# zjwfufu/FateAvatar

Measured on AMD Instinct MI355X. Metric: render+backward frames/sec at 512^2, 100k Gaussians, higher is better.
Workload: dtype f32

## Files before the change

### fateavatar_amd/csrc/fr_common.hpp

```cpp
#pragma once
#include <hip/hip_runtime.h>
#include <stdint.h>
#include <stddef.h>
#include <vector>
#include "../../include/fr_rasterizer.h"

namespace fr {

constexpr int kWave = 64;
constexpr int kTile = 8;
constexpr int kRefTile = 16;
constexpr int kAccumStride = 16;
constexpr int kXcds = 8;
constexpr int kSubWords = 8;
constexpr uint32_t kDensePairsFwd = 1000;
constexpr uint32_t kDensePairsBwd = 1000;
#ifndef FR_PRE_WG
#define FR_PRE_WG 128
#endif
constexpr int kPreWG = FR_PRE_WG;
constexpr uint32_t kBucketCapInit = 64;
constexpr int kSortWaveMax = 256;
constexpr int kSortGroupMax = 2048;
constexpr int kSortRegMax = 4096;
// ... 344 lines not shown
int launch_l1_loss_grad(unsigned long long n, const float* img, const float* gt, float* grad, float* loss, void* workspace,
                        hipStream_t s);
int launch_l1_loss_grad_terms(int n_images, unsigned long long n, float rgb_weight, const float* const* img, const float* const* gt,
                              float* const* grad, float* const* loss, void* const* workspace, hipStream_t s);
void ssim_window(float out[11]);
size_t image_loss_workspace_bytes(int C, int H, int W);
int launch_image_loss_grad(const fr_image_loss_config& cfg, int n_images, int C, int H, int W, const float* const* img,
                           const float* const* gt, float* const* grad, float* const* loss, void* const* workspace, hipStream_t s);
int launch_scaled_sum(int n_src, const float* const* src, float* dst, unsigned long long count, float scale, hipStream_t s);
size_t regularise_workspace_bytes();
int launch_gaussian_regularise(const fr_regularise_config& cfg, int P, const float* scaling, const float* xyz, float* d_scaling,
                               float* d_xyz, float* loss, void* workspace, hipStream_t s);
int launch_multi_copy(int n_seg, float* const* dst, const float* const* src, const unsigned long long* count, hipStream_t s);
int launch_selftest_reduce(const float* in, float* out, hipStream_t s);

#if defined(__HIPCC__)
__device__ __forceinline__ float act_sigmoid(float x) { return 1.0f / (1.0f + expf(-x)); }
__device__ __forceinline__ float act_exp(float x) { return expf(x); }
__device__ __forceinline__ float act_rot_inv_norm(float r, float x, float y, float z)
{
    return 1.0f / fmaxf(sqrtf(r * r + x * x + y * y + z * z), 1e-12f);
}

__device__ __forceinline__ void cov3d_from_scale_rot(float sc0, float sc1, float sc2, float r, float x, float y, float z,
                                                     float scale_modifier, float (&c3)[6])
{
    const float s0 = scale_modifier * sc0, s1 = scale_modifier * sc1, s2 = scale_modifier * sc2;
    const float m00 = s0 * (1.f - 2.f * (y * y + z * z)), m01 = s1 * (2.f * (x * y - r * z)), m02 = s2 * (2.f * (x * z + r * y));
    const float m10 = s0 * (2.f * (x * y + r * z)), m11 = s1 * (1.f - 2.f * (x * x + z * z)), m12 = s2 * (2.f * (y * z - r * x));
    const float m20 = s0 * (2.f * (x * z - r * y)), m21 = s1 * (2.f * (y * z + r * x)), m22 = s2 * (1.f - 2.f * (x * x + y * y));
    c3[0] = m00 * m00 + m01 * m01 + m02 * m02;
    c3[1] = m10 * m00 + m11 * m01 + m12 * m02;
    c3[2] = m20 * m00 + m21 * m01 + m22 * m02;
    c3[3] = m10 * m10 + m11 * m11 + m12 * m12;
    c3[4] = m20 * m10 + m21 * m11 + m22 * m12;
    c3[5] = m20 * m20 + m21 * m21 + m22 * m22;
}
constexpr unsigned kDoneGroups = 16, kDoneStride = 32;
__device__ __forceinline__ bool last_workgroup_of(unsigned* c, unsigned id, unsigned count)
{
    const unsigned groups = count < kDoneGroups ? count : kDoneGroups;
    const unsigned g = id % groups;
    const unsigned members = (count - g + groups - 1u) / groups;
    if (atomicInc(c + g * kDoneStride, members - 1u) != members - 1u) return false;
    return atomicInc(c + kDoneGroups * kDoneStride, groups - 1u) == groups - 1u;
}
__device__ __forceinline__ int lane_id() { return (int)__builtin_amdgcn_mbcnt_hi(~0u, __builtin_amdgcn_mbcnt_lo(~0u, 0u)); }

__device__ __forceinline__ void atomic_add_f32(float* p, float v) { unsafeAtomicAdd(p, v); }

struct CameraRegs {
    float view[16], proj[16], campos[3];
};
__device__ __forceinline__ CameraRegs load_camera(const float* view, const float* proj, const float* campos, int lane)
{
    float x = 0.f;
    if (lane < 16) x = view[lane];
    else if (lane < 32) x = proj[lane - 16];
    else if (lane < 35) x = campos[lane - 32];
    const int xi = __float_as_int(x);
    CameraRegs c;
#pragma unroll
    for (int k = 0; k < 16; k++) {
        c.view[k] = __int_as_float(__builtin_amdgcn_readlane(xi, k));
        c.proj[k] = __int_as_float(__builtin_amdgcn_readlane(xi, 16 + k));
    }
#pragma unroll
    for (int k = 0; k < 3; k++) c.campos[k] = __int_as_float(__builtin_amdgcn_readlane(xi, 32 + k));
    return c;
}

__device__ __forceinline__ float3 xform4x3(const float3 p, const float* m)
{
    return make_float3(m[0] * p.x + m[4] * p.y + m[8] * p.z + m[12], m[1] * p.x + m[5] * p.y + m[9] * p.z + m[13],
                       m[2] * p.x + m[6] * p.y + m[10] * p.z + m[14]);
}
__device__ __forceinline__ float4 xform4x4(const float3 p, const float* m)
{
    return make_float4(m[0] * p.x + m[4] * p.y + m[8] * p.z + m[12], m[1] * p.x + m[5] * p.y + m[9] * p.z + m[13],
                       m[2] * p.x + m[6] * p.y + m[10] * p.z + m[14], m[3] * p.x + m[7] * p.y + m[11] * p.z + m[15]);
}
#endif

}
```

### fateavatar_amd/csrc/fr_preprocess.hip

```cpp
#include "fr_bind_math.hpp"

#ifdef FR_DIAG_PRE_ABLATE
#define FR_PRE_ABLATE(k) (((FR_DIAG_PRE_ABLATE) >> (k)) & 1)
#else
#define FR_PRE_ABLATE(k) false
#endif

#ifdef FR_DIAG_PRE_TRACE
namespace fr {
constexpr unsigned kPreTraceWaves = 16384, kPreTraceSlots = 12;
__device__ unsigned long long g_pre_trace[kPreTraceWaves * kPreTraceSlots];
}
extern "C" int fr_diag_read_pre_trace(void* dst, size_t bytes)
{
    return (int)hipMemcpyFromSymbol(dst, HIP_SYMBOL(fr::g_pre_trace), bytes < sizeof(fr::g_pre_trace) ? bytes : sizeof(fr::g_pre_trace));
}
#define PRE_TR_DECL unsigned long long ptr_acc[::fr::kPreTraceSlots] = {0, 0, 0, 0, 0, 0, 0, 0, 0, 0, 0, 0}, ptr_t = __builtin_readcyclecounter(), ptr_rt0 = __builtin_amdgcn_s_memrealtime()
#define PRE_TR(k) do { const unsigned long long n_ = __builtin_readcyclecounter(); ptr_acc[(k)] += n_ - ptr_t; ptr_t = n_; } while (0)
#define PRE_TR_STORE() do { \
        ptr_acc[11] = (ptr_rt0 << 32) | (__builtin_amdgcn_s_memrealtime() & 0xFFFFFFFFull); \
        const unsigned w_ = (blockIdx.x * kPreWG + threadIdx.x) >> 6; \
        if (lane == 0 && w_ < ::fr::kPreTraceWaves && blockIdx.y == 0) \
            for (unsigned k_ = 0; k_ < ::fr::kPreTraceSlots; k_++) ::fr::g_pre_trace[(size_t)w_ * ::fr::kPreTraceSlots + k_] = ptr_acc[k_]; \
    } while (0)
// ... 98 lines not shown


__device__ __forceinline__ bool footprint_touches_tile(const float4 conic_tau2, const float2 ctr, uint32_t tx, uint32_t ty)
{
    if (!(conic_tau2.w < 3.0e38f)) return true;
    const float A = conic_tau2.x, B = conic_tau2.y, C = conic_tau2.z, t2 = conic_tau2.w;
    const float lox = (float)(tx * kTile) - ctr.x, hix = lox + (float)(kTile - 1);
    const float loy = (float)(ty * kTile) - ctr.y, hiy = loy + (float)(kTile - 1);
    const float qx = lox > 0.f ? lox : (hix < 0.f ? hix : 0.f);
    const float qy = loy > 0.f ? loy : (hiy < 0.f ? hiy : 0.f);
    if (qx == 0.f && qy == 0.f) return true;
    const float dy = fminf(fmaxf(-B * qx * __builtin_amdgcn_rcpf(C), loy), hiy);
    const float dx = fminf(fmaxf(-B * qy * __builtin_amdgcn_rcpf(A), lox), hix);
    const float ax = A * qx * qx, bx = 2.f * B * qx * dy, cx = C * dy * dy;
    const float ay = A * dx * dx, by = 2.f * B * dx * qy, cy = C * qy * qy;
    const float q1 = (ax + bx) + cx, m1 = (ax + fabsf(bx)) + cx;
    const float q2 = (ay + by) + cy, m2 = (ay + fabsf(by)) + cy;
    const bool in1 = qx != 0.f && q1 <= t2 + (4.0e-6f * m1 + 1.0e-4f);
    const bool in2 = qy != 0.f && q2 <= t2 + (4.0e-6f * m2 + 1.0e-4f);
    return in1 || in2;
}

constexpr int kCountUnroll = 4;
constexpr int kCountLdsBytes = 2816 + 3 * kCountUnroll * 256;

#ifndef FR_PRE_SH_DMA
#define FR_PRE_SH_DMA 2
#endif
__device__ __forceinline__ void dma16_to_lds(const void* g, uint32_t lds_byte_address )
{
    asm volatile("s_mov_b32 m0, %0\n\ts_nop 0\n\tglobal_load_lds_dwordx4 %1, off" ::"s"(lds_byte_address), "v"(g) : "memory");
}
#ifndef FR_PRE_ROWS_IN_REGS
#define FR_PRE_ROWS_IN_REGS 1
#endif
__host__ __device__ constexpr int pre_wave_lds_bytes(int M3)
{
#if FR_PRE_ROWS_IN_REGS
    if (M3 == 48) return 256 * M3;
#endif
    return 256 * M3 + kCountLdsBytes;
}

template <bool FWD_ONLY>
__device__ __forceinline__ void preprocess_fwd_body(const PreArgs& a)
{
    extern __shared__ __attribute__((aligned(16))) float s_sh[];
    const int idx = blockIdx.x * blockDim.x + threadIdx.x;
    const int lane = threadIdx.x & 63, wave = threadIdx.x >> 6;
    if (blockIdx.x == 0 && threadIdx.x < sizeof(DeviceCounts) / 4) reinterpret_cast<uint32_t*>(a.counts)[threadIdx.x] = 0u;
    if ((int)(blockIdx.x * kPreWG) >= a.P) return;
    const int M3 = a.M * 3;
    PRE_TR_DECL;
    const CameraRegs cam = load_camera(a.view, a.proj, a.campos, lane);
    const bool live = idx < a.P;
    const int li = live ? idx : 0;
    float3 p_orig;
    float in_sc[3] = {0.f, 0.f, 0.f}, in_rot[4] = {0.f, 0.f, 0.f, 0.f};
    if (a.bound) {
        float bp[3];
        bind_fwd(a.bind, li, bp, in_rot, in_sc);
        p_orig = make_float3(bp[0], bp[1], bp[2]);
        if (live) {
            float* m = const_cast<float*>(a.means3D) + 3 * (size_t)li;
            float* r = const_cast<float*>(a.rotations) + 4 * (size_t)li;
            float* sc = const_cast<float*>(a.scales) + 3 * (size_t)li;
            m[0] = bp[0], m[1] = bp[1], m[2] = bp[2];
            r[0] = in_rot[0], r[1] = in_rot[1], r[2] = in_rot[2], r[3] = in_rot[3];
            sc[0] = in_sc[0], sc[1] = in_sc[1], sc[2] = in_sc[2];
        }
    } else {
        p_orig = make_float3(a.means3D[3 * li], a.means3D[3 * li + 1], a.means3D[3 * li + 2]);
        if (a.scales) in_sc[0] = a.scales[3 * li], in_sc[1] = a.scales[3 * li + 1], in_sc[2] = a.scales[3 * li + 2];
        if (a.rotations)
            in_rot[0] = a.rotations[4 * li], in_rot[1] = a.rotations[4 * li + 1], in_rot[2] = a.rotations[4 * li + 2],
            in_rot[3] = a.rotations[4 * li + 3];
    }
    const float in_opacity = a.opacities[li];
    float in_col[3] = {0.f, 0.f, 0.f};
    if (a.colors_precomp) in_col[0] = a.colors_precomp[3 * li], in_col[1] = a.colors_precomp[3 * li + 1], in_col[2] = a.colors_precomp[3 * li + 2];
    float* const wave_lds = s_sh + (size_t)wave * (pre_wave_lds_bytes(M3) / 4);
    const int wave_first = blockIdx.x * kPreWG + wave * 64;
    const bool rows_in_lds = a.shs && !a.colors_precomp && !FR_PRE_ABLATE(0);
    const bool sh_in_lds = rows_in_lds && __builtin_amdgcn_readfirstlane((int)(FR_PRE_SH_DMA && wave_first + 64 <= a.P)) != 0;
#if FR_PRE_SH_DMA
    if (sh_in_lds) {
        const char* blk = reinterpret_cast<const char*>(a.shs + (size_t)wave_first * M3);
        const int bytes = 256 * M3;
#if FR_PRE_SH_DMA == 2
        const uint32_t lds0 = (uint32_t)__builtin_amdgcn_readfirstlane(
            (int)(uintptr_t)(__attribute__((address_space(3))) void*)wave_lds);
#endif
        for (int off = 0; off < bytes; off += 1024)
            if (off + lane * 16 < bytes) {
#if FR_PRE_SH_DMA == 2
                dma16_to_lds(blk + off + lane * 16, lds0 + (uint32_t)off);
#else
                __builtin_amdgcn_global_load_lds((const __attribute__((address_space(1))) void*)(blk + off + lane * 16),
                                                 (__attribute__((address_space(3))) void*)(reinterpret_cast<char*>(wave_lds) + off), 16, 0, 0);
#endif
            }
    }
#endif
    if (rows_in_lds && !sh_in_lds && live)
        for (int k = 0; k < M3; k++) wave_lds[lane * M3 + k] = a.shs[(size_t)idx * M3 + k];
    uint32_t ref_tiles = 0;
    uint2 rect = make_uint2(0u, 0u);
    float4 cull = make_float4(0.f, 0.f, 0.f, __builtin_inff());
    float2 ctr = make_float2(0.f, 0.f);
    bool alive = false;
    int mr_out = 0;
    float rec_ca = 0.f, rec_cb = 0.f, rec_cc = 0.f, rec_op = 0.f, rec_z = 0.f;
    PRE_TR(0);
    if (idx < a.P) {
        do {
            const float3 p_view = xform4x3(p_orig, cam.view);
            PRE_TR(1);
            if (p_view.z <= 0.2f) break;
            if (FR_PRE_ABLATE(5) && in_opacity > -1e30f) break;

            const float4 p_hom = xform4x4(p_orig, cam.proj);
            const float p_w = 1.0f / (p_hom.w + 0.0000001f);
            const float p_proj_x = p_hom.x * p_w, p_proj_y = p_hom.y * p_w;

            float c3[6];
            if (a.cov3D_precomp) {
                for (int k = 0; k < 6; k++) c3[k] = a.cov3D_precomp[6 * (size_t)idx + k];
            } else {
                float sc0 = in_sc[0], sc1 = in_sc[1], sc2 = in_sc[2];
                float r = in_rot[0], x = in_rot[1], y = in_rot[2], z = in_rot[3];
                if (a.raw) {
                    sc0 = act_exp(sc0), sc1 = act_exp(sc1), sc2 = act_exp(sc2);
                    const float inv = act_rot_inv_norm(r, x, y, z);
// ... 621 lines not shown
```

### fateavatar_amd/csrc/fr_preprocess_bwd.hip

```cpp
#include "fr_bind_math.hpp"

namespace fr {

__constant__ float bSH_C0 = 0.28209479177387814f;
__constant__ float bSH_C1 = 0.4886025119029199f;
__constant__ float bSH_C2[5] = {1.0925484305920792f, -1.0925484305920792f, 0.31539156525252005f,
                                -1.0925484305920792f, 0.5462742152960396f};
__constant__ float bSH_C3[7] = {-0.5900435899266435f, 2.890611442640554f, -0.4570457994644658f, 0.3731763325901154f,
                                -0.4570457994644658f, 1.445305721320277f,  -0.5900435899266435f};

struct PreBwdArgs {
    int P, D, M, W, H, raw;
    float tan_fovx, tan_fovy, focal_x, focal_y, scale_modifier;
    const float* means3D;
    const float* scales;
    const float* rotations;
    const float* shs;
    const float* cov3D_precomp;
    const float* view;
    const float* proj;
    const float* campos;
    const int* radii;
    GeomView g;
    fr_grads out;
    float* grad_accum;
    float* denom;
    float* overflow_out;
    const DeviceCounts* counts;
    uint32_t acc;
    int bound;
    BindArgs bind;
    BindGrads bg;
};

enum { G_MEANS2D = 0, G_COLORS, G_OPACITY, G_MEANS3D, G_COV3D, G_SH, G_SCALES, G_ROTATIONS };

__device__ __forceinline__ void put(float* p, float v, bool add) { *p = add ? *p + v : v; }

__device__ __forceinline__ void store3(float* p, size_t i, float a, float b, float c, bool add)
{
    if (!p) return;
    if (add) a += p[3 * i], b += p[3 * i + 1], c += p[3 * i + 2];
    p[3 * i] = a, p[3 * i + 1] = b, p[3 * i + 2] = c;
}

template <bool PLANES>
__device__ __forceinline__ void preprocess_bwd_one(const PreBwdArgs& a, const CameraRegs& cam, const int radius,
                                                   const int idx, float* row)
{
    const size_t i = (size_t)idx;
    const int Mc = a.M;
    const auto adds = [&](int k) { return ((a.acc >> k) & 1u) != 0u; };
    if (!(radius > 0)) {
        if (row)
            for (int k = 0; k < Mc * 3; k++) row[k] = 0.f;
        if (!adds(G_MEANS2D)) store3(a.out.dL_dmeans2D, i, 0.f, 0.f, 0.f, false);
        if (!adds(G_COLORS)) store3(a.out.dL_dcolors, i, 0.f, 0.f, 0.f, false);
        if (a.out.dL_dopacity && !adds(G_OPACITY)) a.out.dL_dopacity[i] = 0.f;
        if (!adds(G_MEANS3D)) store3(a.out.dL_dmeans3D, i, 0.f, 0.f, 0.f, false);
        if (a.out.dL_dcov3D && !adds(G_COV3D))
            for (int k = 0; k < 6; k++) a.out.dL_dcov3D[6 * i + k] = 0.f;
        if (a.out.dL_dsh && !row && !adds(G_SH))
            for (int k = 0; k < Mc * 3; k++) a.out.dL_dsh[i * Mc * 3 + k] = 0.f;
        if (!adds(G_SCALES)) store3(a.out.dL_dscales, i, 0.f, 0.f, 0.f, false);
        if (a.out.dL_drotations && !adds(G_ROTATIONS))
            for (int k = 0; k < 4; k++) a.out.dL_drotations[4 * i + k] = 0.f;
        if (a.bound) bind_bwd_zero(idx, a.bg);
        return;
    }
    float old_m3[3] = {0.f, 0.f, 0.f}, old_sc[3] = {0.f, 0.f, 0.f}, old_q[4] = {0.f, 0.f, 0.f, 0.f}, old_op = 0.f;
    if (a.acc) {
        if (adds(G_MEANS3D) && a.out.dL_dmeans3D)
            for (int k = 0; k < 3; k++) old_m3[k] = a.out.dL_dmeans3D[3 * i + k];
        if (adds(G_SCALES) && a.out.dL_dscales)
            for (int k = 0; k < 3; k++) old_sc[k] = a.out.dL_dscales[3 * i + k];
        if (adds(G_ROTATIONS) && a.out.dL_drotations)
            for (int k = 0; k < 4; k++) old_q[k] = a.out.dL_drotations[4 * i + k];
        if (adds(G_OPACITY) && a.out.dL_dopacity) old_op = a.out.dL_dopacity[i];
    }
    float acc[12];
    {
        float4* row4 = reinterpret_cast<float4*>(a.g.accum + i * kAccumStride);
        const float4 r0 = row4[0], r1 = row4[1], r2 = row4[2];
        row4[0] = row4[1] = row4[2] = make_float4(0.f, 0.f, 0.f, 0.f);
        acc[0] = r0.x, acc[1] = r0.y, acc[2] = r0.z, acc[3] = r0.w, acc[4] = r1.x, acc[5] = r1.y, acc[6] = r1.z,
        acc[7] = r1.w, acc[8] = r2.x, acc[9] = r2.y, acc[10] = r2.z, acc[11] = r2.w;
    }
    const float3 mean = make_float3(a.means3D[3 * idx], a.means3D[3 * idx + 1], a.means3D[3 * idx + 2]);
    const float* vm = cam.view;
    float q_r = 0.f, q_x = 0.f, q_y = 0.f, q_z = 0.f, rot_inv = 1.0f;
    float sc[3] = {0.f, 0.f, 0.f};
    float c3[6];
    if (a.scales) {
        q_r = a.rotations[4 * idx], q_x = a.rotations[4 * idx + 1], q_y = a.rotations[4 * idx + 2], q_z = a.rotations[4 * idx + 3];
        sc[0] = a.scales[3 * idx], sc[1] = a.scales[3 * idx + 1], sc[2] = a.scales[3 * idx + 2];
        if (a.raw) {
            sc[0] = act_exp(sc[0]), sc[1] = act_exp(sc[1]), sc[2] = act_exp(sc[2]);
            rot_inv = act_rot_inv_norm(q_r, q_x, q_y, q_z);
            q_r *= rot_inv, q_x *= rot_inv, q_y *= rot_inv, q_z *= rot_inv;
        }
    }
    if (a.cov3D_precomp) {
        for (int k = 0; k < 6; k++) c3[k] = a.cov3D_precomp[6 * i + k];
    } else {
        cov3d_from_scale_rot(sc[0], sc[1], sc[2], q_r, q_x, q_y, q_z, a.scale_modifier, c3);
    }

    float3 t = xform4x3(mean, vm);
    const float limx = 1.3f * a.tan_fovx, limy = 1.3f * a.tan_fovy;
    const float txtz = t.x / t.z, tytz = t.y / t.z;
    t.x = fminf(limx, fmaxf(-limx, txtz)) * t.z;
    t.y = fminf(limy, fmaxf(-limy, tytz)) * t.z;
    const float x_grad_mul = txtz < -limx || txtz > limx ? 0 : 1;
    const float y_grad_mul = tytz < -limy || tytz > limy ? 0 : 1;
    const float h_x = a.focal_x, h_y = a.focal_y;
    const float j00 = h_x / t.z, j02 = -(h_x * t.x) / (t.z * t.z);
    const float j11 = h_y / t.z, j12 = -(h_y * t.y) / (t.z * t.z);
    float T0[3], T1[3];
    for (int w = 0; w < 3; w++) {
        const float W0 = vm[4 * w], W1 = vm[4 * w + 1], W2 = vm[4 * w + 2];
        T0[w] = W0 * j00 + W1 * 0.0f + W2 * j02;
        T1[w] = W0 * 0.0f + W1 * j11 + W2 * j12;
    }
    const float V[3][3] = {{c3[0], c3[1], c3[2]}, {c3[1], c3[3], c3[4]}, {c3[2], c3[4], c3[5]}};
    float A0[3], A1[3];
    for (int c = 0; c < 3; c++) {
        A0[c] = T0[0] * V[0][c] + T0[1] * V[1][c] + T0[2] * V[2][c];
        A1[c] = T1[0] * V[0][c] + T1[1] * V[1][c] + T1[2] * V[2][c];
    }
    float ca = A0[0] * T0[0] + A0[1] * T0[1] + A0[2] * T0[2];
    const float cb = A1[0] * T0[0] + A1[1] * T0[1] + A1[2] * T0[2];
    float cc = A1[0] * T1[0] + A1[1] * T1[1] + A1[2] * T1[2];
    ca += 0.3f;
    cc += 0.3f;
    const float denom = ca * cc - cb * cb;
    const float det_inv = 1.f / denom;
    const float4 co = make_float4(cc * det_inv, -cb * det_inv, ca * det_inv, a.g.opacity_act[idx]);
    const float g2x = acc[ACC_MX] * (0.5f * a.W);
    const float g2y = acc[ACC_MY] * (0.5f * a.H);
    const float dcx = -0.5f * acc[ACC_CA], dcy = -0.5f * acc[ACC_CB], dcz = -0.5f * acc[ACC_CC];
    const float dop = (co.w != 0.f) ? acc[ACC_OP] / co.w : 0.f;
    float dcol[3] = {acc[ACC_R], acc[ACC_G], acc[ACC_B]};
    store3(a.out.dL_dmeans2D, i, g2x, g2y, 0.f, adds(G_MEANS2D));
    if (!a.counts->overflow) {
        if (a.grad_accum) a.grad_accum[i] += sqrtf(g2x * g2x + g2y * g2y);
        if (a.denom) a.denom[i] += 1.0f;
    }
    store3(a.out.dL_dcolors, i, dcol[0], dcol[1], dcol[2], adds(G_COLORS));
    if (a.out.dL_dopacity) a.out.dL_dopacity[i] = old_op + (a.raw ? dop * co.w * (1.0f - co.w) : dop);

    float dL_da = 0, dL_db = 0, dL_dc = 0;
    const float denom2inv = 1.0f / ((denom * denom) + 0.0000001f);
    float dcov[6] = {0, 0, 0, 0, 0, 0};
    if (denom2inv != 0) {
        dL_da = denom2inv * (-cc * cc * dcx + 2 * cb * cc * dcy + (denom - ca * cc) * dcz);
        dL_dc = denom2inv * (-ca * ca * dcz + 2 * ca * cb * dcy + (denom - ca * cc) * dcx);
        dL_db = denom2inv * 2 * (cb * cc * dcx - (denom + 2 * cb * cb) * dcy + ca * cb * dcz);
        dcov[0] = (T0[0] * T0[0] * dL_da + T0[0] * T1[0] * dL_db + T1[0] * T1[0] * dL_dc);
        dcov[3] = (T0[1] * T0[1] * dL_da + T0[1] * T1[1] * dL_db + T1[1] * T1[1] * dL_dc);
        dcov[5] = (T0[2] * T0[2] * dL_da + T0[2] * T1[2] * dL_db + T1[2] * T1[2] * dL_dc);
        dcov[1] = 2 * T0[0] * T0[1] * dL_da + (T0[0] * T1[1] + T0[1] * T1[0]) * dL_db + 2 * T1[0] * T1[1] * dL_dc;
        dcov[2] = 2 * T0[0] * T0[2] * dL_da + (T0[0] * T1[2] + T0[2] * T1[0]) * dL_db + 2 * T1[0] * T1[2] * dL_dc;
        dcov[4] = 2 * T0[2] * T0[1] * dL_da + (T0[1] * T1[2] + T0[2] * T1[1]) * dL_db + 2 * T1[1] * T1[2] * dL_dc;
    }
    if (a.out.dL_dcov3D)
        for (int k = 0; k < 6; k++) put(a.out.dL_dcov3D + 6 * i + k, dcov[k], adds(G_COV3D));

    float dT0[3], dT1[3];
    for (int c = 0; c < 3; c++) {
        const float tv0 = T0[0] * V[c][0] + T0[1] * V[c][1] + T0[2] * V[c][2];
        const float tv1 = T1[0] * V[c][0] + T1[1] * V[c][1] + T1[2] * V[c][2];
        dT0[c] = 2 * tv0 * dL_da + tv1 * dL_db;
        dT1[c] = 2 * tv1 * dL_dc + tv0 * dL_db;
    }
    const float dL_dJ00 = vm[0] * dT0[0] + vm[4] * dT0[1] + vm[8] * dT0[2];
    const float dL_dJ02 = vm[2] * dT0[0] + vm[6] * dT0[1] + vm[10] * dT0[2];
    const float dL_dJ11 = vm[1] * dT1[0] + vm[5] * dT1[1] + vm[9] * dT1[2];
    const float dL_dJ12 = vm[2] * dT1[0] + vm[6] * dT1[1] + vm[10] * dT1[2];
    const float tz = 1.f / t.z, tz2 = tz * tz, tz3 = tz2 * tz;
    const float dL_dtx = x_grad_mul * -h_x * tz2 * dL_dJ02;
    const float dL_dty = y_grad_mul * -h_y * tz2 * dL_dJ12;
    const float dL_dtz = -h_x * tz2 * dL_dJ00 - h_y * tz2 * dL_dJ11 + (2 * h_x * t.x) * tz3 * dL_dJ02 + (2 * h_y * t.y) * tz3 * dL_dJ12;
    float dmx = vm[0] * dL_dtx + vm[1] * dL_dty + vm[2] * dL_dtz;
    float dmy = vm[4] * dL_dtx + vm[5] * dL_dty + vm[6] * dL_dtz;
    float dmz = vm[8] * dL_dtx + vm[9] * dL_dty + vm[10] * dL_dtz;

    {
        const float* proj = cam.proj;
        const float4 m_hom = xform4x4(mean, proj);
        const float m_w = 1.0f / (m_hom.w + 0.0000001f);
        const float mul1 = (proj[0] * mean.x + proj[4] * mean.y + proj[8] * mean.z + proj[12]) * m_w * m_w;
        const float mul2 = (proj[1] * mean.x + proj[5] * mean.y + proj[9] * mean.z + proj[13]) * m_w * m_w;
        const float px = (proj[0] * m_w - proj[3] * mul1) * g2x + (proj[1] * m_w - proj[3] * mul2) * g2y;
        const float py = (proj[4] * m_w - proj[7] * mul1) * g2x + (proj[5] * m_w - proj[7] * mul2) * g2y;
        const float pz = (proj[8] * m_w - proj[11] * mul1) * g2x + (proj[9] * m_w - proj[11] * mul2) * g2y;
        dmx += px, dmy += py, dmz += pz;
    }

    if (a.shs) {
        const float dox = mean.x - cam.campos[0], doy = mean.y - cam.campos[1], doz = mean.z - cam.campos[2];
        const float len = sqrtf(dox * dox + doy * doy + doz * doz);
        const float x = dox / len, y = doy / len, z = doz / len;
        const uint8_t cl = a.g.clamped[idx];
        float dRGB[3];
        for (int c = 0; c < 3; c++) dRGB[c] = dcol[c] * (((cl >> c) & 1) ? 0 : 1);
        const float* dd = a.g.dcolor_ddir + i * 9;
        const float dRGBdx[3] = {dd[0], dd[1], dd[2]}, dRGBdy[3] = {dd[3], dd[4], dd[5]}, dRGBdz[3] = {dd[6], dd[7], dd[8]};
        const int deg = a.D;
        const int used = (deg + 1) * (deg + 1);
        auto write_row = [&](float* dsh, const bool dsh_adds) {
#define DSH(k, c, v_) put(dsh + (k) * 3 + (c), (v_), dsh_adds)
            for (int c = 0; c < 3; c++) {
                DSH(0, c, bSH_C0 * dRGB[c]);
                if (deg > 0) {
                    DSH(1, c, (-bSH_C1 * y) * dRGB[c]);
                    DSH(2, c, (bSH_C1 * z) * dRGB[c]);
                    DSH(3, c, (-bSH_C1 * x) * dRGB[c]);
                    if (deg > 1) {
                        const float xx = x * x, yy = y * y, zz = z * z;
                        const float xy = x * y, yz = y * z, xz = x * z;
                        DSH(4, c, (bSH_C2[0] * xy) * dRGB[c]);
                        DSH(5, c, (bSH_C2[1] * yz) * dRGB[c]);
                        DSH(6, c, (bSH_C2[2] * (2.f * zz - xx - yy)) * dRGB[c]);
                        DSH(7, c, (bSH_C2[3] * xz) * dRGB[c]);
                        DSH(8, c, (bSH_C2[4] * (xx - yy)) * dRGB[c]);
                        if (deg > 2) {
                            DSH(9, c, (bSH_C3[0] * y * (3.f * xx - yy)) * dRGB[c]);
                            DSH(10, c, (bSH_C3[1] * xy * z) * dRGB[c]);
                            DSH(11, c, (bSH_C3[2] * y * (4.f * zz - xx - yy)) * dRGB[c]);
                            DSH(12, c, (bSH_C3[3] * z * (2.f * zz - 3.f * xx - 3.f * yy)) * dRGB[c]);
                            DSH(13, c, (bSH_C3[4] * x * (4.f * zz - xx - yy)) * dRGB[c]);
                            DSH(14, c, (bSH_C3[5] * z * (xx - yy)) * dRGB[c]);
                            DSH(15, c, (bSH_C3[6] * x * (xx - 3.f * yy)) * dRGB[c]);
                        }
                    }
                }
            }
            if (!dsh_adds)
                for (int k = used; k < Mc; k++) dsh[k * 3] = 0.f, dsh[k * 3 + 1] = 0.f, dsh[k * 3 + 2] = 0.f;
#undef DSH
        };
        if (row) write_row(row, false);
        else if (a.out.dL_dsh) write_row(a.out.dL_dsh + i * Mc * 3, adds(G_SH));
        const float ddx = dRGBdx[0] * dRGB[0] + dRGBdx[1] * dRGB[1] + dRGBdx[2] * dRGB[2];
        const float ddy = dRGBdy[0] * dRGB[0] + dRGBdy[1] * dRGB[1] + dRGBdy[2] * dRGB[2];
        const float ddz = dRGBdz[0] * dRGB[0] + dRGBdz[1] * dRGB[1] + dRGBdz[2] * dRGB[2];
        const float sum2 = dox * dox + doy * doy + doz * doz;
        const float invsum32 = 1.0f / sqrtf(sum2 * sum2 * sum2);
        dmx += ((+sum2 - dox * dox) * ddx - doy * dox * ddy - doz * dox * ddz) * invsum32;
        dmy += (-dox * doy * ddx + (sum2 - doy * doy) * ddy - doz * doy * ddz) * invsum32;
        dmz += (-dox * doz * ddx - doy * doz * ddy + (sum2 - doz * doz) * ddz) * invsum32;
    } else if (a.out.dL_dsh && !row && !adds(G_SH)) {
        for (int k = 0; k < Mc * 3; k++) a.out.dL_dsh[i * Mc * 3 + k] = 0.f;
    }
    if (PLANES) {
        const float dz = acc[ACC_Z];
        dmx += dz * vm[2], dmy += dz * vm[6], dmz += dz * vm[10];
    }
    store3(a.out.dL_dmeans3D, i, old_m3[0] + dmx, old_m3[1] + dmy, old_m3[2] + dmz, false);
    const float g_mean[3] = {dmx, dmy, dmz};
    float g_scl[3] = {0.f, 0.f, 0.f}, g_rot[4] = {0.f, 0.f, 0.f, 0.f};

    if (a.scales) {
        const float r = q_r, x = q_x, y = q_y, z = q_z;
        const float s[3] = {a.scale_modifier * sc[0], a.scale_modifier * sc[1], a.scale_modifier * sc[2]};
        const float Rc[3][3] = {{1.f - 2.f * (y * y + z * z), 2.f * (x * y - r * z), 2.f * (x * z + r * y)},
                                {2.f * (x * y + r * z), 1.f - 2.f * (x * x + z * z), 2.f * (y * z - r * x)},
                                {2.f * (x * z - r * y), 2.f * (y * z + r * x), 1.f - 2.f * (x * x + y * y)}};
        const float dS[3][3] = {{dcov[0], 0.5f * dcov[1], 0.5f * dcov[2]},
                                {0.5f * dcov[1], dcov[3], 0.5f * dcov[4]},
                                {0.5f * dcov[2], 0.5f * dcov[4], dcov[5]}};
        float dM[3][3];
        for (int c = 0; c < 3; c++)
            for (int w = 0; w < 3; w++)
                dM[c][w] = (s[w] * Rc[0][w] * 2.0f) * dS[c][0] + (s[w] * Rc[1][w] * 2.0f) * dS[c][1] + (s[w] * Rc[2][w] * 2.0f) * dS[c][2];
        float dMt[3][3];
        for (int c = 0; c < 3; c++)
            for (int w = 0; w < 3; w++) dMt[c][w] = dM[w][c];
        const float dsx = Rc[0][0] * dMt[0][0] + Rc[1][0] * dMt[0][1] + Rc[2][0] * dMt[0][2];
        const float dsy = Rc[0][1] * dMt[1][0] + Rc[1][1] * dMt[1][1] + Rc[2][1] * dMt[1][2];
        const float dsz = Rc[0][2] * dMt[2][0] + Rc[1][2] * dMt[2][1] + Rc[2][2] * dMt[2][2];
        g_scl[0] = a.raw ? dsx * sc[0] : dsx, g_scl[1] = a.raw ? dsy * sc[1] : dsy, g_scl[2] = a.raw ? dsz * sc[2] : dsz;
        store3(a.out.dL_dscales, i, old_sc[0] + g_scl[0], old_sc[1] + g_scl[1], old_sc[2] + g_scl[2], false);
        for (int w = 0; w < 3; w++) dMt[0][w] *= s[0], dMt[1][w] *= s[1], dMt[2][w] *= s[2];
#define Dm(c_, r_) dMt[c_][r_]
        if (a.out.dL_drotations || a.bound) {
            float dq[4];
            dq[0] = 2 * z * (Dm(0, 1) - Dm(1, 0)) + 2 * y * (Dm(2, 0) - Dm(0, 2)) + 2 * x * (Dm(1, 2) - Dm(2, 1));
            dq[1] = 2 * y * (Dm(1, 0) + Dm(0, 1)) + 2 * z * (Dm(2, 0) + Dm(0, 2)) + 2 * r * (Dm(1, 2) - Dm(2, 1)) - 4 * x * (Dm(2, 2) + Dm(1, 1));
            dq[2] = 2 * x * (Dm(1, 0) + Dm(0, 1)) + 2 * r * (Dm(2, 0) - Dm(0, 2)) + 2 * z * (Dm(1, 2) + Dm(2, 1)) - 4 * y * (Dm(2, 2) + Dm(0, 0));
            dq[3] = 2 * r * (Dm(0, 1) - Dm(1, 0)) + 2 * x * (Dm(2, 0) + Dm(0, 2)) + 2 * y * (Dm(1, 2) + Dm(2, 1)) - 4 * z * (Dm(1, 1) + Dm(0, 0));
            if (a.raw) {
                const float dot = r * dq[0] + x * dq[1] + y * dq[2] + z * dq[3];
                dq[0] = (dq[0] - r * dot) * rot_inv;
                dq[1] = (dq[1] - x * dot) * rot_inv;
// ... 4 lines not shown
                for (int k = 0; k < 4; k++) a.out.dL_drotations[4 * i + k] = old_q[k] + dq[k];
            for (int k = 0; k < 4; k++) g_rot[k] = dq[k];
        }
#undef Dm
    } else {
        if (!adds(G_SCALES)) store3(a.out.dL_dscales, i, 0.f, 0.f, 0.f, false);
        if (a.out.dL_drotations && !adds(G_ROTATIONS))
            for (int k = 0; k < 4; k++) a.out.dL_drotations[4 * i + k] = 0.f;
    }
    if (a.bound) bind_bwd(a.bind, idx, g_mean, g_rot, g_scl, a.bg);
}

template <bool ADD>
__device__ __forceinline__ void unstage_rows_t(float* __restrict__ dst, const float* src, int stride, int rows, int row_len, int lane)
{
    const int total = rows * row_len;
    const unsigned magic = (unsigned)((0x100000000ull + (unsigned)row_len - 1u) / (unsigned)row_len);
    constexpr int kBatch = ADD ? 6 : 1;
    for (int base = lane * 4; base < total; base += 64 * 4 * kBatch) {
        float4 o[kBatch];
        if (ADD) {
#pragma unroll
            for (int u = 0; u < kBatch; u++) {
                const int c = base + u * 64 * 4;
                o[u] = make_float4(0.f, 0.f, 0.f, 0.f);
                if (c + 3 < total) {
                    o[u] = *reinterpret_cast<const float4*>(dst + c);
                } else {
                    if (c < total) o[u].x = dst[c];
                    if (c + 1 < total) o[u].y = dst[c + 1];
                    if (c + 2 < total) o[u].z = dst[c + 2];
                }
            }
        }
#pragma unroll
        for (int u = 0; u < kBatch; u++) {
            const int c = base + u * 64 * 4;
            if (c >= total) break;
            float v[4];
#pragma unroll
            for (int k = 0; k < 4; k++) {
                const int e = c + k;
                const int r = (int)__umulhi((unsigned)e, magic);
                v[k] = (e < total) ? src[r * stride + (e - r * row_len)] : 0.f;
            }
            if (ADD) v[0] += o[u].x, v[1] += o[u].y, v[2] += o[u].z, v[3] += o[u].w;
            if (c + 3 < total) *reinterpret_cast<float4*>(dst + c) = make_float4(v[0], v[1], v[2], v[3]);
            else
                for (int k = 0; k < 4; k++)
                    if (c + k < total) dst[c + k] = v[k];
        }
    }
}
__device__ __forceinline__ void unstage_rows(float* __restrict__ dst, const float* src, int stride, int rows, int row_len, int lane,
                                             bool add)
{
    if (add) unstage_rows_t<true>(dst, src, stride, rows, row_len, lane);
    else unstage_rows_t<false>(dst, src, stride, rows, row_len, lane);
}

#ifndef FR_PREBWD_WAVES
#define FR_PREBWD_WAVES 4
#endif
constexpr int kPreBwdWaves = FR_PREBWD_WAVES;

template <bool PLANES>
__device__ __forceinline__ void preprocess_bwd_body(const PreBwdArgs& a)
{
    extern __shared__ __attribute__((aligned(16))) float s_rows[];
    if ((int)(blockIdx.x * blockDim.x) >= a.P) return;
    const int idx = blockIdx.x * blockDim.x + threadIdx.x;
    const int lane = threadIdx.x & 63, wave = threadIdx.x >> 6;
    if (a.overflow_out && blockIdx.x == 0 && threadIdx.x == 0) *a.overflow_out = a.counts->overflow ? 1.0f : 0.0f;
    const int M3 = a.M * 3, stride = M3 | 1;
    const int wave_first = blockIdx.x * (64 * kPreBwdWaves) + wave * 64;
    const int rows = min(64, a.P - wave_first);
    const bool staged = a.shs != nullptr && a.out.dL_dsh != nullptr;
    float* w_rows = s_rows + (size_t)wave * 64 * stride;
    const CameraRegs cam = load_camera(a.view, a.proj, a.campos, lane);
    const int radius = idx < a.P ? a.radii[idx] : 0;
    if (idx < a.P) preprocess_bwd_one<PLANES>(a, cam, radius, idx, staged ? w_rows + lane * stride : nullptr);
    __syncthreads();
    if (staged && rows > 0) unstage_rows(a.out.dL_dsh + (size_t)wave_first * M3, w_rows, stride, rows, M3, lane, ((a.acc >> G_SH) & 1u) != 0u);
}

__global__ void __launch_bounds__(64 * kPreBwdWaves) k_preprocess_bwd(PreBwdArgs a) { preprocess_bwd_body<false>(a); }
__global__ void __launch_bounds__(64 * kPreBwdWaves) k_preprocess_bwd_batch(BatchOf<PreBwdArgs> b) { preprocess_bwd_body<false>(b.v[blockIdx.y]); }
__global__ void __launch_bounds__(64 * kPreBwdWaves) k_preprocess_bwd_planes(PreBwdArgs a) { preprocess_bwd_body<true>(a); }
__global__ void __launch_bounds__(64 * kPreBwdWaves) k_preprocess_bwd_planes_batch(BatchOf<PreBwdArgs> b) { preprocess_bwd_body<true>(b.v[blockIdx.y]); }

int launch_blend_backward(int n, const BackwardCall* calls, const GeomView* g, const ImageView* v, bool planes, hipStream_t s, bool debug);

int launch_backward(int n, const BackwardCall* calls, hipStream_t s)
{
    GeomView g[kMaxBatch];
    ImageView v[kMaxBatch];
    PreBwdArgs args[kMaxBatch];
    bool capturing = false, debug = false, planes = false;
    for (int k = 0; k < n; k++) capturing = note_capture(calls[k].h, s) || capturing;
    for (int k = 0; k < n; k++) {
        const fr_aux* aux = calls[k].prm->aux;
        planes = planes || ((calls[k].prm->flags & FR_FLAG_DEPTH_ALPHA) && aux && (aux->dL_ddepth || aux->dL_dalpha));
    }
    size_t lds = 0;
    uint32_t blocks = 0;
    const int wg = 64 * kPreBwdWaves;
    for (int k = 0; k < n; k++) {
        fr_handle_impl* h = calls[k].h;
        const fr_params& prm = *calls[k].prm;
        const fr_inputs& in = *calls[k].in;
        const int P = prm.P;
        g[k] = GeomView::make(calls[k].geometry, (size_t)P);
        if (!capturing && h->have_last_bwd && h->last_bwd_stream != s) FR_HIP(hipStreamWaitEvent(s, h->bwd_done, 0));
        {
            int rc0 = ensure_accum(h, (size_t)P, s);
            if (rc0) return rc0;
            g[k].accum = h->accum;
        }
        v[k] = ImageView::make(const_cast<void*>(calls[k].image), prm.W, prm.H);
        debug = debug || prm.debug != 0;
        PreBwdArgs& a = args[k];
        a.P = P, a.D = prm.D, a.M = prm.M, a.W = prm.W, a.H = prm.H;
        a.raw = (prm.flags & FR_FLAG_RAW_ACTIVATIONS) ? 1 : 0;
        a.tan_fovx = prm.tan_fovx, a.tan_fovy = prm.tan_fovy;
        a.focal_y = prm.H / (2.0f * prm.tan_fovy);
        a.focal_x = prm.W / (2.0f * prm.tan_fovx);
        a.scale_modifier = prm.scale_modifier;
        a.means3D = in.means3D, a.scales = in.scales, a.rotations = in.rotations, a.shs = in.shs;
        a.cov3D_precomp = in.cov3D_precomp, a.view = in.viewmatrix, a.proj = in.projmatrix, a.campos = in.campos;
        a.radii = calls[k].radii, a.g = g[k], a.out = *calls[k].grads;
        a.grad_accum = prm.aux ? prm.aux->grad_accum : nullptr;
        a.denom = prm.aux ? prm.aux->denom : nullptr;
        a.overflow_out = prm.aux ? prm.aux->overflow_out : nullptr;
        a.counts = v[k].counts;
        a.acc = ((uint32_t)prm.flags >> FR_FLAG_ACCUMULATE_SHIFT) & 0xFFu;
        a.bound = (prm.aux && prm.aux->binding) ? 1 : 0;
        if (a.bound) {
            a.bind = bind_args(*prm.aux->binding);
            a.bg = BindGrads{prm.aux->d_verts, prm.aux->d_offset, prm.aux->d_rotation, prm.aux->d_scaling, prm.aux->d_local_xyz};
        } else {
            a.bind = BindArgs{};
            a.bg = BindGrads{};
        }
        const size_t l = (in.shs && calls[k].grads->dL_dsh) ? (size_t)kPreBwdWaves * 64 * ((prm.M * 3) | 1) * sizeof(float) : 0;
        lds = l > lds ? l : lds;
        blocks = max(blocks, (uint32_t)((P + wg - 1) / wg));
    }
    int rc = launch_blend_backward(n, calls, g, v, planes, s, debug);
    if (rc) return rc;
    {
        StageScope sc(calls[0].h, ST_PREPROCESS_BWD, s);
        if (planes) launch_views(k_preprocess_bwd_planes, k_preprocess_bwd_planes_batch, n, args, blocks, (uint32_t)wg, lds, s);
        else launch_views(k_preprocess_bwd, k_preprocess_bwd_batch, n, args, blocks, (uint32_t)wg, lds, s);
    }
    FR_HIP(hipGetLastError());
    if (!capturing)
        for (int k = 0; k < n; k++) {
            fr_handle_impl* h = calls[k].h;
            FR_HIP(hipEventRecord(h->bwd_done, s));
            h->last_bwd_stream = s, h->have_last_bwd = true;
        }
    if (debug) FR_HIP(hipStreamSynchronize(s));
    return FR_OK;
}

}
```

Before: 21060.

## Hoist preprocess-backward global loads upfront and vectorize SH gradient row staging

Preprocess backward now issues every per-Gaussian global load (radius, accum row, means, rotation, scales, opacity, clamped flags, dcolor_ddir, grad_accum, denom, old gradients) in one fetch stage before the camera broadcast, so their latencies overlap instead of being serialized through the compute. The camera load is split into a request and a broadcast, also in forward preprocess, so other loads can be in flight in between. SH gradient rows with M3 divisible by 4 are written to LDS as float4 with a padded stride and copied out to global with float4 accesses. This raises register pressure from holding all inputs, and loads are now issued for inactive (radius 0) Gaussians as well.

```diff
diff --git a/fateavatar_amd/csrc/fr_common.hpp b/fateavatar_amd/csrc/fr_common.hpp
--- a/fateavatar_amd/csrc/fr_common.hpp
+++ b/fateavatar_amd/csrc/fr_common.hpp
@@ -420,12 +420,15 @@
 struct CameraRegs {
     float view[16], proj[16], campos[3];
 };
-__device__ __forceinline__ CameraRegs load_camera(const float* view, const float* proj, const float* campos, int lane)
-{
+__device__ __forceinline__ float camera_request(const float* view, const float* proj, const float* campos, int lane)
+{
+    const float* p = lane < 16 ? view + lane : (lane < 32 ? proj + (lane - 16) : campos + (lane - 32));
     float x = 0.f;
-    if (lane < 16) x = view[lane];
-    else if (lane < 32) x = proj[lane - 16];
-    else if (lane < 35) x = campos[lane - 32];
+    if (lane < 35) x = *p;
+    return x;
+}
+__device__ __forceinline__ CameraRegs camera_broadcast(float x)
+{
     const int xi = __float_as_int(x);
     CameraRegs c;
 #pragma unroll
@@ -437,6 +440,10 @@
     for (int k = 0; k < 3; k++) c.campos[k] = __int_as_float(__builtin_amdgcn_readlane(xi, 32 + k));
     return c;
 }
+__device__ __forceinline__ CameraRegs load_camera(const float* view, const float* proj, const float* campos, int lane)
+{
+    return camera_broadcast(camera_request(view, proj, campos, lane));
+}
 
 __device__ __forceinline__ float3 xform4x3(const float3 p, const float* m)
 {
diff --git a/fateavatar_amd/csrc/fr_preprocess.hip b/fateavatar_amd/csrc/fr_preprocess.hip
--- a/fateavatar_amd/csrc/fr_preprocess.hip
+++ b/fateavatar_amd/csrc/fr_preprocess.hip
@@ -174,7 +174,7 @@
     if ((int)(blockIdx.x * kPreWG) >= a.P) return;
     const int M3 = a.M * 3;
     PRE_TR_DECL;
-    const CameraRegs cam = load_camera(a.view, a.proj, a.campos, lane);
+    const float cam_x = camera_request(a.view, a.proj, a.campos, lane);
     const bool live = idx < a.P;
     const int li = live ? idx : 0;
     float3 p_orig;
@@ -201,6 +201,7 @@
     const float in_opacity = a.opacities[li];
     float in_col[3] = {0.f, 0.f, 0.f};
     if (a.colors_precomp) in_col[0] = a.colors_precomp[3 * li], in_col[1] = a.colors_precomp[3 * li + 1], in_col[2] = a.colors_precomp[3 * li + 2];
+    const CameraRegs cam = camera_broadcast(cam_x);
     float* const wave_lds = s_sh + (size_t)wave * (pre_wave_lds_bytes(M3) / 4);
     const int wave_first = blockIdx.x * kPreWG + wave * 64;
     const bool rows_in_lds = a.shs && !a.colors_precomp && !FR_PRE_ABLATE(0);
diff --git a/fateavatar_amd/csrc/fr_preprocess_bwd.hip b/fateavatar_amd/csrc/fr_preprocess_bwd.hip
--- a/fateavatar_amd/csrc/fr_preprocess_bwd.hip
+++ b/fateavatar_amd/csrc/fr_preprocess_bwd.hip
@@ -44,15 +44,98 @@
     p[3 * i] = a, p[3 * i + 1] = b, p[3 * i + 2] = c;
 }
 
+__host__ __device__ constexpr bool prebwd_rows_by16(int M3) { return M3 % 4 == 0 && M3 <= 48; }
+__host__ __device__ constexpr int prebwd_row_stride(int M3)
+{
+    return prebwd_rows_by16(M3) ? (((M3 / 4) & 1) ? M3 : M3 + 4) : (M3 | 1);
+}
+
+struct PreBwdIn {
+    int radius;
+    float mean[3], q[4], sc[3], c3[6];
+    float opacity;
+    uint32_t cl;
+    float dd[9];
+    float4 r0, r1, r2;
+    uint32_t overflow;
+    float ga, dn;
+    float old_m3[3], old_sc[3], old_q[4], old_op;
+};
+
+template <class T> using GlobalPtr = const __attribute__((address_space(1))) T*;
+template <class T> __device__ __forceinline__ GlobalPtr<T> as_global(const T* p) { return (GlobalPtr<T>)p; }
+typedef float PreBwdF4 __attribute__((ext_vector_type(4)));
+
+__device__ __forceinline__ void preprocess_bwd_fetch(const PreBwdArgs& a, const int li, PreBwdIn& in)
+{
+    const size_t i = (size_t)li;
+    const auto adds = [&](int k) { return ((a.acc >> k) & 1u) != 0u; };
+    const int* radii_ = a.radii;
+    const DeviceCounts* counts_ = a.counts;
+    const float *accum_ = a.g.accum, *means3D_ = a.means3D, *scales_ = a.scales, *rotations_ = a.rotations, *cov3D_ = a.cov3D_precomp;
+    const float *opacity_act_ = a.g.opacity_act, *dcolor_ddir_ = a.g.dcolor_ddir, *shs = a.shs;
+    const uint8_t* clamped_ = a.g.clamped;
+    const float *grad_accum_ = a.grad_accum, *denom_ = a.denom;
+    asm volatile("" : "+s"(radii_), "+s"(counts_), "+s"(accum_), "+s"(means3D_), "+s"(scales_), "+s"(rotations_), "+s"(cov3D_),
+                 "+s"(opacity_act_), "+s"(dcolor_ddir_), "+s"(shs), "+s"(clamped_), "+s"(grad_accum_), "+s"(denom_));
+    const auto radii = as_global(radii_);
+    const auto counts = as_global(counts_);
+    const auto accum = as_global(accum_), means3D = as_global(means3D_), scales = as_global(scales_), rotations = as_global(rotations_);
+    const auto cov3D = as_global(cov3D_), opacity_act = as_global(opacity_act_), dcolor_ddir = as_global(dcolor_ddir_);
+    const auto clamped = as_global(clamped_);
+    const auto grad_accum = as_global(grad_accum_), denom = as_global(denom_);
+    in.radius = radii[li];
+    in.overflow = counts->overflow;
+    const GlobalPtr<PreBwdF4> row4 = (GlobalPtr<PreBwdF4>)(accum + i * kAccumStride);
+    const PreBwdF4 r0 = row4[0], r1 = row4[1], r2 = row4[2];
+    in.r0 = make_float4(r0.x, r0.y, r0.z, r0.w), in.r1 = make_float4(r1.x, r1.y, r1.z, r1.w), in.r2 = make_float4(r2.x, r2.y, r2.z, r2.w);
+    for (int k = 0; k < 3; k++) in.mean[k] = means3D[3 * i + k];
+    for (int k = 0; k < 4; k++) in.q[k] = 0.f;
+    for (int k = 0; k < 3; k++) in.sc[k] = 0.f;
+    for (int k = 0; k < 6; k++) in.c3[k] = 0.f;
+    if (scales) {
+        for (int k = 0; k < 4; k++) in.q[k] = rotations[4 * i + k];
+        for (int k = 0; k < 3; k++) in.sc[k] = scales[3 * i + k];
+    }
+    if (cov3D)
+        for (int k = 0; k < 6; k++) in.c3[k] = cov3D[6 * i + k];
+    in.opacity = opacity_act[li];
+    in.cl = 0u;
+    for (int k = 0; k < 9; k++) in.dd[k] = 0.f;
+    if (shs) {
+        in.cl = clamped[li];
+        for (int k = 0; k < 9; k++) in.dd[k] = dcolor_ddir[i * 9 + k];
+    }
+    in.ga = in.dn = 0.f;
+    if (grad_accum) in.ga = grad_accum[i];
+    if (denom) in.dn = denom[i];
+    for (int k = 0; k < 3; k++) in.old_m3[k] = 0.f, in.old_sc[k] = 0.f;
+    for (int k = 0; k < 4; k++) in.old_q[k] = 0.f;
+    in.old_op = 0.f;
+    if (a.acc) {
+        if (adds(G_MEANS3D) && a.out.dL_dmeans3D)
+            for (int k = 0; k < 3; k++) in.old_m3[k] = a.out.dL_dmeans3D[3 * i + k];
+        if (adds(G_SCALES) && a.out.dL_dscales)
+            for (int k = 0; k < 3; k++) in.old_sc[k] = a.out.dL_dscales[3 * i + k];
+        if (adds(G_ROTATIONS) && a.out.dL_drotations)
+            for (int k = 0; k < 4; k++) in.old_q[k] = a.out.dL_drotations[4 * i + k];
+        if (adds(G_OPACITY) && a.out.dL_dopacity) in.old_op = a.out.dL_dopacity[i];
+    }
+}
+
 template <bool PLANES>
-__device__ __forceinline__ void preprocess_bwd_one(const PreBwdArgs& a, const CameraRegs& cam, const int radius,
-                                                   const int idx, float* row)
+__device__ __forceinline__ void preprocess_bwd_one(const PreBwdArgs& a, const CameraRegs& cam, const PreBwdIn& in,
+                                                   const int idx, float* row, const bool by16)
 {
     const size_t i = (size_t)idx;
     const int Mc = a.M;
+    const int radius = in.radius;
     const auto adds = [&](int k) { return ((a.acc >> k) & 1u) != 0u; };
     if (!(radius > 0)) {
-        if (row)
+        if (row && by16) {
+            float4* r4 = reinterpret_cast<float4*>(row);
+            for (int k = 0; k < (Mc * 3) / 4; k++) r4[k] = make_float4(0.f, 0.f, 0.f, 0.f);
+        } else if (row)
             for (int k = 0; k < Mc * 3; k++) row[k] = 0.f;
         if (!adds(G_MEANS2D)) store3(a.out.dL_dmeans2D, i, 0.f, 0.f, 0.f, false);
         if (!adds(G_COLORS)) store3(a.out.dL_dcolors, i, 0.f, 0.f, 0.f, false);
@@ -68,32 +151,24 @@
         if (a.bound) bind_bwd_zero(idx, a.bg);
         return;
     }
-    float old_m3[3] = {0.f, 0.f, 0.f}, old_sc[3] = {0.f, 0.f, 0.f}, old_q[4] = {0.f, 0.f, 0.f, 0.f}, old_op = 0.f;
-    if (a.acc) {
-        if (adds(G_MEANS3D) && a.out.dL_dmeans3D)
-            for (int k = 0; k < 3; k++) old_m3[k] = a.out.dL_dmeans3D[3 * i + k];
-        if (adds(G_SCALES) && a.out.dL_dscales)
-            for (int k = 0; k < 3; k++) old_sc[k] = a.out.dL_dscales[3 * i + k];
-        if (adds(G_ROTATIONS) && a.out.dL_drotations)
-            for (int k = 0; k < 4; k++) old_q[k] = a.out.dL_drotations[4 * i + k];
-        if (adds(G_OPACITY) && a.out.dL_dopacity) old_op = a.out.dL_dopacity[i];
-    }
+    const float old_m3[3] = {in.old_m3[0], in.old_m3[1], in.old_m3[2]}, old_sc[3] = {in.old_sc[0], in.old_sc[1], in.old_sc[2]};
+    const float old_q[4] = {in.old_q[0], in.old_q[1], in.old_q[2], in.old_q[3]}, old_op = in.old_op;
     float acc[12];
     {
         float4* row4 = reinterpret_cast<float4*>(a.g.accum + i * kAccumStride);
-        const float4 r0 = row4[0], r1 = row4[1], r2 = row4[2];
+        const float4 r0 = in.r0, r1 = in.r1, r2 = in.r2;
         row4[0] = row4[1] = row4[2] = make_float4(0.f, 0.f, 0.f, 0.f);
         acc[0] = r0.x, acc[1] = r0.y, acc[2] = r0.z, acc[3] = r0.w, acc[4] = r1.x, acc[5] = r1.y, acc[6] = r1.z,
         acc[7] = r1.w, acc[8] = r2.x, acc[9] = r2.y, acc[10] = r2.z, acc[11] = r2.w;
     }
-    const float3 mean = make_float3(a.means3D[3 * idx], a.means3D[3 * idx + 1], a.means3D[3 * idx + 2]);
+    const float3 mean = make_float3(in.mean[0], in.mean[1], in.mean[2]);
     const float* vm = cam.view;
     float q_r = 0.f, q_x = 0.f, q_y = 0.f, q_z = 0.f, rot_inv = 1.0f;
     float sc[3] = {0.f, 0.f, 0.f};
     float c3[6];
     if (a.scales) {
-        q_r = a.rotations[4 * idx], q_x = a.rotations[4 * idx + 1], q_y = a.rotations[4 * idx + 2], q_z = a.rotations[4 * idx + 3];
-        sc[0] = a.scales[3 * idx], sc[1] = a.scales[3 * idx + 1], sc[2] = a.scales[3 * idx + 2];
+        q_r = in.q[0], q_x = in.q[1], q_y = in.q[2], q_z = in.q[3];
+        sc[0] = in.sc[0], sc[1] = in.sc[1], sc[2] = in.sc[2];
         if (a.raw) {
             sc[0] = act_exp(sc[0]), sc[1] = act_exp(sc[1]), sc[2] = act_exp(sc[2]);
             rot_inv = act_rot_inv_norm(q_r, q_x, q_y, q_z);
@@ -101,7 +176,7 @@
         }
     }
     if (a.cov3D_precomp) {
-        for (int k = 0; k < 6; k++) c3[k] = a.cov3D_precomp[6 * i + k];
+        for (int k = 0; k < 6; k++) c3[k] = in.c3[k];
     } else {
         cov3d_from_scale_rot(sc[0], sc[1], sc[2], q_r, q_x, q_y, q_z, a.scale_modifier, c3);
     }
@@ -135,16 +210,16 @@
     cc += 0.3f;
     const float denom = ca * cc - cb * cb;
     const float det_inv = 1.f / denom;
-    const float4 co = make_float4(cc * det_inv, -cb * det_inv, ca * det_inv, a.g.opacity_act[idx]);
+    const float4 co = make_float4(cc * det_inv, -cb * det_inv, ca * det_inv, in.opacity);
     const float g2x = acc[ACC_MX] * (0.5f * a.W);
     const float g2y = acc[ACC_MY] * (0.5f * a.H);
     const float dcx = -0.5f * acc[ACC_CA], dcy = -0.5f * acc[ACC_CB], dcz = -0.5f * acc[ACC_CC];
     const float dop = (co.w != 0.f) ? acc[ACC_OP] / co.w : 0.f;
     float dcol[3] = {acc[ACC_R], acc[ACC_G], acc[ACC_B]};
     store3(a.out.dL_dmeans2D, i, g2x, g2y, 0.f, adds(G_MEANS2D));
-    if (!a.counts->overflow) {
-        if (a.grad_accum) a.grad_accum[i] += sqrtf(g2x * g2x + g2y * g2y);
-        if (a.denom) a.denom[i] += 1.0f;
+    if (!in.overflow) {
+        if (a.grad_accum) a.grad_accum[i] = in.ga + sqrtf(g2x * g2x + g2y * g2y);
+        if (a.denom) a.denom[i] = in.dn + 1.0f;
     }
     store3(a.out.dL_dcolors, i, dcol[0], dcol[1], dcol[2], adds(G_COLORS));
     if (a.out.dL_dopacity) a.out.dL_dopacity[i] = old_op + (a.raw ? dop * co.w * (1.0f - co.w) : dop);
@@ -201,10 +276,10 @@
         const float dox = mean.x - cam.campos[0], doy = mean.y - cam.campos[1], doz = mean.z - cam.campos[2];
         const float len = sqrtf(dox * dox + doy * doy + doz * doz);
         const float x = dox / len, y = doy / len, z = doz / len;
-        const uint8_t cl = a.g.clamped[idx];
+        const uint32_t cl = in.cl;
         float dRGB[3];
         for (int c = 0; c < 3; c++) dRGB[c] = dcol[c] * (((cl >> c) & 1) ? 0 : 1);
-        const float* dd = a.g.dcolor_ddir + i * 9;
+        const float* dd = in.dd;
         const float dRGBdx[3] = {dd[0], dd[1], dd[2]}, dRGBdy[3] = {dd[3], dd[4], dd[5]}, dRGBdz[3] = {dd[6], dd[7], dd[8]};
         const int deg = a.D;
         const int used = (deg + 1) * (deg + 1);
@@ -240,7 +315,40 @@
                 for (int k = used; k < Mc; k++) dsh[k * 3] = 0.f, dsh[k * 3 + 1] = 0.f, dsh[k * 3 + 2] = 0.f;
 #undef DSH
         };
-        if (row) write_row(row, false);
+        auto write_row_by16 = [&](float* dsh) {
+            float f[16] = {0.f, 0.f, 0.f, 0.f, 0.f, 0.f, 0.f, 0.f, 0.f, 0.f, 0.f, 0.f, 0.f, 0.f, 0.f, 0.f};
+            f[0] = bSH_C0;
+            if (deg > 0) {
+                f[1] = -bSH_C1 * y, f[2] = bSH_C1 * z, f[3] = -bSH_C1 * x;
+                if (deg > 1) {
+                    const float xx = x * x, yy = y * y, zz = z * z;
+                    const float xy = x * y, yz = y * z, xz = x * z;
+                    f[4] = bSH_C2[0] * xy, f[5] = bSH_C2[1] * yz, f[6] = bSH_C2[2] * (2.f * zz - xx - yy);
+                    f[7] = bSH_C2[3] * xz, f[8] = bSH_C2[4] * (xx - yy);
+                    if (deg > 2) {
+                        f[9] = bSH_C3[0] * y * (3.f * xx - yy), f[10] = bSH_C3[1] * xy * z;
+                        f[11] = bSH_C3[2] * y * (4.f * zz - xx - yy), f[12] = bSH_C3[3] * z * (2.f * zz - 3.f * xx - 3.f * yy);
+                        f[13] = bSH_C3[4] * x * (4.f * zz - xx - yy), f[14] = bSH_C3[5] * z * (xx - yy);
+                        f[15] = bSH_C3[6] * x * (xx - 3.f * yy);
+                    }
+                }
+            }
+            float4* d4 = reinterpret_cast<float4*>(dsh);
+            const int pieces = (Mc * 3) / 4;
+#pragma unroll
+            for (int j = 0; j < 12; j++) {
+                if (j >= pieces) break;
+                float v[4];
+#pragma unroll
+                for (int t = 0; t < 4; t++) {
+                    const int k = (4 * j + t) / 3, c = (4 * j + t) % 3;
+                    v[t] = k < used ? f[k] * dRGB[c] : 0.f;
+                }
+                d4[j] = make_float4(v[0], v[1], v[2], v[3]);
+            }
+        };
+        if (row && by16) write_row_by16(row);
+        else if (row) write_row(row, false);
         else if (a.out.dL_dsh) write_row(a.out.dL_dsh + i * Mc * 3, adds(G_SH));
         const float ddx = dRGBdx[0] * dRGB[0] + dRGBdx[1] * dRGB[1] + dRGBdx[2] * dRGB[2];
         const float ddy = dRGBdy[0] * dRGB[0] + dRGBdy[1] * dRGB[1] + dRGBdy[2] * dRGB[2];
@@ -351,11 +459,43 @@
         }
     }
 }
+template <bool ADD>
+__device__ __forceinline__ void unstage_rows_by16_t(float* __restrict__ dst, const float* src, int stride, int rows, int row_len, int lane)
+{
+    const int total = rows * row_len;
+    const unsigned magic = (unsigned)((0x100000000ull + (unsigned)row_len - 1u) / (unsigned)row_len);
+    constexpr int kBatch = ADD ? 6 : 1;
+    for (int base = lane * 4; base < total; base += 64 * 4 * kBatch) {
+        float4 o[kBatch];
+        if (ADD) {
+#pragma unroll
+            for (int u = 0; u < kBatch; u++) {
+                const int c = base + u * 64 * 4;
+                o[u] = make_float4(0.f, 0.f, 0.f, 0.f);
+                if (c < total) o[u] = *reinterpret_cast<const float4*>(dst + c);
+            }
+        }
+#pragma unroll
+        for (int u = 0; u < kBatch; u++) {
+            const int c = base + u * 64 * 4;
+            if (c >= total) break;
+            const int r = (int)__umulhi((unsigned)c, magic);
+            float4 v = *reinterpret_cast<const float4*>(src + r * stride + (c - r * row_len));
+            if (ADD) v.x += o[u].x, v.y += o[u].y, v.z += o[u].z, v.w += o[u].w;
+            *reinterpret_cast<float4*>(dst + c) = v;
+        }
+    }
+}
 __device__ __forceinline__ void unstage_rows(float* __restrict__ dst, const float* src, int stride, int rows, int row_len, int lane,
                                              bool add)
 {
-    if (add) unstage_rows_t<true>(dst, src, stride, rows, row_len, lane);
-    else unstage_rows_t<false>(dst, src, stride, rows, row_len, lane);
+    if (prebwd_rows_by16(row_len)) {
+        if (add) unstage_rows_by16_t<true>(dst, src, stride, rows, row_len, lane);
+        else unstage_rows_by16_t<false>(dst, src, stride, rows, row_len, lane);
+    } else {
+        if (add) unstage_rows_t<true>(dst, src, stride, rows, row_len, lane);
+        else unstage_rows_t<false>(dst, src, stride, rows, row_len, lane);
+    }
 }
 
 #ifndef FR_PREBWD_WAVES
@@ -370,15 +510,19 @@
     if ((int)(blockIdx.x * blockDim.x) >= a.P) return;
     const int idx = blockIdx.x * blockDim.x + threadIdx.x;
     const int lane = threadIdx.x & 63, wave = threadIdx.x >> 6;
-    if (a.overflow_out && blockIdx.x == 0 && threadIdx.x == 0) *a.overflow_out = a.counts->overflow ? 1.0f : 0.0f;
-    const int M3 = a.M * 3, stride = M3 | 1;
+    const int M3 = a.M * 3, stride = prebwd_row_stride(M3);
     const int wave_first = blockIdx.x * (64 * kPreBwdWaves) + wave * 64;
     const int rows = min(64, a.P - wave_first);
     const bool staged = a.shs != nullptr && a.out.dL_dsh != nullptr;
     float* w_rows = s_rows + (size_t)wave * 64 * stride;
-    const CameraRegs cam = load_camera(a.view, a.proj, a.campos, lane);
-    const int radius = idx < a.P ? a.radii[idx] : 0;
-    if (idx < a.P) preprocess_bwd_one<PLANES>(a, cam, radius, idx, staged ? w_rows + lane * stride : nullptr);
+    PreBwdIn in;
+    preprocess_bwd_fetch(a, min(idx, a.P - 1), in);
+    const float cam_x = camera_request(a.view, a.proj, a.campos, lane);
+    asm volatile("" ::: "memory");
+    const CameraRegs cam = camera_broadcast(cam_x);
+    asm volatile("" : "+v"(in.cl), "+v"(in.ga), "+v"(in.dn), "+v"(in.opacity), "+v"(in.radius));
+    if (a.overflow_out && blockIdx.x == 0 && threadIdx.x == 0) *a.overflow_out = in.overflow ? 1.0f : 0.0f;
+    if (idx < a.P) preprocess_bwd_one<PLANES>(a, cam, in, idx, staged ? w_rows + lane * stride : nullptr, prebwd_rows_by16(M3));
     __syncthreads();
     if (staged && rows > 0) unstage_rows(a.out.dL_dsh + (size_t)wave_first * M3, w_rows, stride, rows, M3, lane, ((a.acc >> G_SH) & 1u) != 0u);
 }
@@ -441,7 +585,7 @@
             a.bind = BindArgs{};
             a.bg = BindGrads{};
         }
-        const size_t l = (in.shs && calls[k].grads->dL_dsh) ? (size_t)kPreBwdWaves * 64 * ((prm.M * 3) | 1) * sizeof(float) : 0;
+        const size_t l = (in.shs && calls[k].grads->dL_dsh) ? (size_t)kPreBwdWaves * 64 * prebwd_row_stride(prm.M * 3) * sizeof(float) : 0;
         lds = l > lds ? l : lds;
         blocks = max(blocks, (uint32_t)((P + wg - 1) / wg));
     }
```

After: 22080, median of 6. +4.9%, better.
